# OpenDriveLab/kai0

Hardware: AMD Instinct MI355X
Metric: train samples/sec pi0.5 full FT (higher is better)
Workload: dtype bf16; 1 GPU; pi0.5 full fine-tune bf16, batch 32 per MI355X, 3-cam 224x224 (BASELINE.json configs[1]); global_batch=32, seq_len=1018, parallelism=dp1

## Files before the change

### include/kai0hip.h

```cpp
#ifndef KAI0HIP_H
#define KAI0HIP_H

#include <stdint.h>

#ifdef __cplusplus
extern "C" {
#endif

typedef void* kai0_stream_t;

const char* kai0_last_error(void);
int kai0_abi_version(void);
int kai0_device_info(int device, int* n_cu, int* lds_bytes, char* arch_name64);

typedef struct kai0_gemm_desc {
    const void* A;
    const void* B;
    void* C;
    int32_t M, N, K;
    int32_t a_kc, b_kc;
    int64_t lda, ldb, ldc;
    int32_t batch, batch_inner;
    int64_t sA1, sA2, sB1, sB2, sC1, sC2;
    int32_t a_rpb, b_rpb, c_rpb, _pad0;
// ... 5 lines not shown
    int32_t out_f32;
    void* pre_out;
    const void* gate;
    int32_t gate_rpb;
    int32_t accumulate;
    int64_t gate_ld;
    const void* residual;
    int64_t ldr;
    int64_t sR1, sR2;
    int32_t split_k;
    int32_t c_nontemporal;
    void* workspace;
    int64_t workspace_bytes;
    const void* aux1;
    const void* aux2;
    int32_t nseg, _pad2;
    struct {
        void* dst;
        int64_t ld;
        int32_t n_begin, _pad;
    } seg[3];
    const float* rowvec;
    int64_t rv_s1, rv_s2, rv_ld;
    const void* B2;
    void* pre_out2;
    void* norm_out;
    const void* norm_w;
    const void* norm_b;
    float norm_eps;
    int32_t norm_kind;
    const void* rope_cos;
    const void* rope_sin;
    int32_t rope_half, rope_n_end;
    int32_t persist, general_epilogue, small_w8, _pad3;
} kai0_gemm_desc;

int kai0_gemm_bf16(const kai0_gemm_desc* d, kai0_stream_t stream);
int kai0_gemm_desc_size(void);

#define KAI0_GEMM_LOOP_PLAIN2 0
#define KAI0_GEMM_LOOP_PLAIN4 1
#define KAI0_GEMM_LOOP_QUADRANT 2
#define KAI0_GEMM_LOOP_RING 3
#define KAI0_GEMM_LOOP_PERSISTENT 4
typedef struct kai0_gemm_plan_t {
    int32_t tile;
    int32_t waves;
    int32_t loop;
    int32_t tiles_m, tiles_n;
    int32_t k_chunk;
    int32_t simple_epilogue;
    int32_t _pad;
} kai0_gemm_plan_t;
int kai0_gemm_plan(const kai0_gemm_desc* d, kai0_gemm_plan_t* out);
int kai0_gemm_plan_size(void);

typedef struct kai0_skinny_seg {
    void* dst;
    int64_t ld;
    int32_t n_begin, n_end;
    int32_t rope, _pad;
} kai0_skinny_seg;

typedef struct kai0_skinny_desc {
    const void* A;
    const void* W;
    int64_t lda, ldw;
    int32_t M, N, K;
    int32_t pair_stride, mode, split_k;
    int32_t a_rpb, c_rpb;
    int64_t a_bs, a_off, c_bs, c_off;
    kai0_skinny_seg seg[3];
    int32_t nseg, gate_rpb;
    const void* gate;
    int64_t gate_ld;
    const void* residual;
    int64_t ldr;
    const float* rope_cos;
    const float* rope_sin;
    int32_t rope_half;
    int32_t w_packed;
    void* workspace;
    int64_t workspace_bytes;
    const float* mod;
    int64_t mod_ld;
// ... 233 lines not shown
```

### kai0_amd/_lib.py

```python

from __future__ import annotations

import ctypes as C
import os
import pathlib

_HERE = pathlib.Path(__file__).resolve().parent
LIB_PATH = _HERE / "lib" / "libkai0hip.so"
ABI_VERSION = 2

c_p = C.c_void_p
c_i = C.c_int
c_i64 = C.c_int64
c_f = C.c_float


class GemmSeg(C.Structure):
    _fields_ = [("dst", c_p), ("ld", c_i64), ("n_begin", C.c_int32), ("_pad", C.c_int32)]


class GemmDesc(C.Structure):

    _fields_ = [
        ("A", c_p), ("B", c_p), ("C", c_p),
        ("M", C.c_int32), ("N", C.c_int32), ("K", C.c_int32),
        ("a_kc", C.c_int32), ("b_kc", C.c_int32),
        ("lda", c_i64), ("ldb", c_i64), ("ldc", c_i64),
        ("batch", C.c_int32), ("batch_inner", C.c_int32),
        ("sA1", c_i64), ("sA2", c_i64), ("sB1", c_i64), ("sB2", c_i64), ("sC1", c_i64), ("sC2", c_i64),
        ("a_rpb", C.c_int32), ("b_rpb", C.c_int32), ("c_rpb", C.c_int32), ("_pad0", C.c_int32),
        ("a_bs", c_i64), ("a_off", c_i64), ("b_bs", c_i64), ("b_off", c_i64), ("c_bs", c_i64), ("c_off", c_i64),
        ("bias", c_p), ("bias_f32", C.c_int32), ("scale", c_f),
        ("act", C.c_int32), ("out_f32", C.c_int32),
        ("pre_out", c_p), ("gate", c_p), ("gate_rpb", C.c_int32), ("accumulate", C.c_int32),
        ("gate_ld", c_i64), ("residual", c_p), ("ldr", c_i64), ("sR1", c_i64), ("sR2", c_i64),
        ("split_k", C.c_int32), ("c_nontemporal", C.c_int32), ("workspace", c_p), ("workspace_bytes", c_i64),
        ("aux1", c_p), ("aux2", c_p),
        ("nseg", C.c_int32), ("_pad2", C.c_int32), ("seg", GemmSeg * 3),
        ("rowvec", c_p), ("rv_s1", c_i64), ("rv_s2", c_i64), ("rv_ld", c_i64),
        ("B2", c_p), ("pre_out2", c_p),
        ("norm_out", c_p), ("norm_w", c_p), ("norm_b", c_p), ("norm_eps", C.c_float), ("norm_kind", C.c_int32),
        ("rope_cos", c_p), ("rope_sin", c_p), ("rope_half", C.c_int32), ("rope_n_end", C.c_int32),
        ("persist", C.c_int32), ("general_epilogue", C.c_int32), ("small_w8", C.c_int32), ("_pad3", C.c_int32),
    ]


class GemmPlan(C.Structure):

    _fields_ = [("tile", C.c_int32), ("waves", C.c_int32), ("loop", C.c_int32), ("tiles_m", C.c_int32), ("tiles_n", C.c_int32),
                ("k_chunk", C.c_int32), ("simple_epilogue", C.c_int32), ("_pad", C.c_int32)]


GEMM_LOOPS = ("plain2", "plain4", "quadrant", "ring", "persistent")


class AttnDesc(C.Structure):

    _fields_ = [
        ("Q", c_p), ("K", c_p), ("V", c_p), ("O", c_p), ("P", c_p), ("qcode", c_p), ("kcode", c_p),
        ("rows", C.c_int32), ("Sk", C.c_int32), ("HD", C.c_int32), ("H", C.c_int32), ("q0", C.c_int32),
        ("batch", C.c_int32), ("batch_inner", C.c_int32), ("_pad0", C.c_int32),
        ("ldq", c_i64), ("ldk", c_i64), ("ldv", c_i64), ("ldo", c_i64), ("ldp", c_i64),
        ("sQ1", c_i64), ("sQ2", c_i64), ("sK1", c_i64), ("sK2", c_i64), ("sV1", c_i64), ("sV2", c_i64),
        ("sO1", c_i64), ("sO2", c_i64), ("sP", c_i64), ("qcode_ld", c_i64), ("kcode_ld", c_i64),
        ("scale", c_f), ("online", C.c_int32), ("lse", c_p), ("s_lse", c_i64),
    ]


class AttnBwdDesc(C.Structure):

    _fields_ = [
        ("dO", c_p), ("O", c_p), ("Q", c_p), ("K", c_p), ("V", c_p), ("lse", c_p), ("qcode", c_p), ("kcode", c_p),
        ("P", c_p), ("dS", c_p), ("dQ", c_p),
        ("batch", C.c_int32), ("rows", C.c_int32), ("Sk", C.c_int32), ("HD", C.c_int32), ("H", C.c_int32), ("_pad0", C.c_int32),
        ("ldo", c_i64), ("ldk", c_i64), ("ldv", c_i64), ("ldp", c_i64), ("sO", c_i64), ("sK", c_i64), ("sV", c_i64), ("sP", c_i64),
        ("s_lse", c_i64), ("qcode_ld", c_i64), ("kcode_ld", c_i64),
        ("scale", c_f), ("_pad1", C.c_int32),
    ]


class SkinnySeg(C.Structure):
    _fields_ = [("dst", c_p), ("ld", c_i64), ("n_begin", C.c_int32), ("n_end", C.c_int32), ("rope", C.c_int32),
                ("_pad", C.c_int32)]
# ... 185 lines not shown
```

### kai0_amd/csrc/gemm_bf16.hip

```cpp
#include "common.h"
#include "../../include/kai0hip.h"
#include <stdlib.h>
#include <algorithm>
#include <atomic>
#include <type_traits>

namespace {

constexpr int BK = 64;

#ifdef KAI0_ABLATE
#define KAI0_ABL(p) ((p).ablate)
#else
#define KAI0_ABL(p) 0
#endif

struct RowMap {
    int32_t rpb;
    int64_t bs, off;
    __device__ __forceinline__ int64_t operator()(int r) const {
        if (rpb == 0) return r;
        const int q = r / rpb;
        return (int64_t)q * bs + (r - q * rpb) + off;
    }
};

struct GemmArgs {
    const bf16_t* A;
    const bf16_t* B;
    void* C;
    int M, N, K;
    int64_t lda, ldb, ldc;
    int batch_inner;
    int64_t sA1, sA2, sB1, sB2, sC1, sC2;
    RowMap amap, bmap, cmap;
    const void* bias;
    int bias_f32;
    float scale;
    int act;
    int out_f32;
    bf16_t* pre_out;
    const bf16_t* aux1;
    const bf16_t* aux2;
    const bf16_t* gate;
    int gate_rpb;
    int accumulate;
    int64_t gate_ld;
    const bf16_t* residual;
    int64_t ldr, sR1, sR2;
    int tiles_m, tiles_n;
    int ablate;
    int nt_c;
    int simple_epi;
    int nt_pre;
    const float* rowvec;
    int64_t rv_s1, rv_s2, rv_ld;
    int nseg;
    bf16_t* seg_dst[3];
    int64_t seg_ld[3];
    int seg_begin[3];
    float* ws;
    int split_k, k_chunk;
    const bf16_t* B2;
    bf16_t* pre_out2;
    bf16_t* norm_out;
    const void* norm_w;
    const bf16_t* norm_b;
    float norm_eps;
    int norm_kind;
    const bf16_t* rope_cos;
    const bf16_t* rope_sin;
    int rope_half, rope_n_end;
};

typedef __attribute__((ext_vector_type(4))) int i32x4_t;
constexpr uint32_t OOB = 0x80000000u;
__device__ __forceinline__ void glds16(__amdgpu_buffer_rsrc_t rsrc, uint32_t voff, char* lds_dst_wave_uniform) {
    __builtin_amdgcn_raw_ptr_buffer_load_lds(rsrc, (LDS_PTR(void))lds_dst_wave_uniform, 16, (int)voff, 0, 0, 0);
}


__device__ __forceinline__ void store_pre8(bf16_t* dst, bf16x8 v, int nt) {
    if (nt) __builtin_nontemporal_store(v, reinterpret_cast<bf16x8*>(dst));
    else *reinterpret_cast<bf16x8*>(dst) = v;
}

// ... 1102 lines not shown
            lds_barrier();
            quad(I0{}, I0{});
            lds_barrier();
            read_b(tb, 1);
            __builtin_amdgcn_sched_barrier(0);
            issue_half(false, 1, t + 1);
            asm volatile("s_waitcnt vmcnt(8)" ::: "memory");
            lds_barrier();
            quad(I0{}, I1{});
            lds_barrier();
            read_a(ta, 1);
            __builtin_amdgcn_sched_barrier(0);
            issue_half(false, 0, t + 2);
            lds_barrier();
            quad(I1{}, I1{});
            lds_barrier();
            read_b(tb, 0);
            __builtin_amdgcn_sched_barrier(0);
            issue_half(true, 1, t + 2);
            asm volatile("s_waitcnt vmcnt(6)" ::: "memory");
            lds_barrier();
            quad(I1{}, I0{});
            lds_barrier();
        }
        asm volatile("s_waitcnt vmcnt(0)" ::: "memory");
        if (grp == 0) lds_barrier();
        lds_barrier();

        PS_STAMP(1);
        const int m0c = m0, n0c = n0;
        int nn = -1;
        unsigned raw = 0;
        if (tid == 0 && nxt >= 0) raw = draw();
        if (nxt >= 0) {
            setup(nxt);
            prologue_issue();
        }
        const int ccol = n0c + wn * 64 + (lane & 7) * 8;
        const bool col_ok = ccol < ((p.N + 7) & ~7);
        const bool fused_fast = p.act >= 2 && p.act <= 5 && p.bias == nullptr && p.gate == nullptr && p.residual == nullptr && !p.accumulate &&
                                !p.out_f32 && p.nseg == 0 && (p.act == 4 || p.scale == 1.0f) && (p.act != 3 || p.pre_out != nullptr);
        const bool simple_fast = SIMPLE_EPILOGUE_APPLIES(p.simple_epi, p.act, p.split_k, p.gate, p.out_f32, p.scale, p.cmap.rpb, p.N);
        auto to_slab = [&](int ti) {
            __builtin_amdgcn_wave_barrier();
#pragma unroll
            for (int j = 0; j < 4; ++j)
#pragma unroll
                for (int r = 0; r < 4; ++r) slab[(4 * g + r) * 64 + j * 16 + l15] = acc[ti][j][r];
            asm volatile("s_waitcnt lgkmcnt(0)" ::: "memory");
            __builtin_amdgcn_wave_barrier();
        };
        if (pair) {
            const int ocol = (n0c >> 1) + wn * 32 + (lane & 3) * 8;
            const bool ocol_ok = ocol < (p.N >> 1);
            bf16_t* cb = reinterpret_cast<bf16_t*>(p.C);
#pragma unroll
            for (int ti = 0; ti < MT; ++ti) {
                to_slab(ti);
                const int row = m0c + wm * 128 + ti * 16 + (lane >> 2);
                const float* sp = slab + (lane >> 2) * 64 + (lane & 3) * 8;
                const f32x4 g0 = *reinterpret_cast<const f32x4*>(sp), g1 = *reinterpret_cast<const f32x4*>(sp + 4);
                const f32x4 u0 = *reinterpret_cast<const f32x4*>(sp + 32), u1 = *reinterpret_cast<const f32x4*>(sp + 36);
                if (row < p.M && ocol_ok) {
                    const float gv[8] = {g0[0], g0[1], g0[2], g0[3], g1[0], g1[1], g1[2], g1[3]};
                    const float uv[8] = {u0[0], u0[1], u0[2], u0[3], u1[0], u1[1], u1[2], u1[3]};
                    bf16x8 gb, ub, hb;
#pragma unroll
                    for (int e = 0; e < 8; e += 2) {
                        const f32x2 gr = rbf2(f32x2{gv[e], gv[e + 1]}), ur = rbf2(f32x2{uv[e], uv[e + 1]});
                        const f32x2 hv = rbf2(gelu_tanh2(gr)) * ur;
                        gb[e] = f2bf(gr[0]); gb[e + 1] = f2bf(gr[1]);
                        ub[e] = f2bf(ur[0]); ub[e + 1] = f2bf(ur[1]);
                        hb[e] = f2bf(hv[0]); hb[e + 1] = f2bf(hv[1]);
                    }
                    const int64_t o = p.cmap(row) * p.ldc + ocol;
                    *reinterpret_cast<bf16x8*>(cb + o) = hb;
                    if (p.pre_out != nullptr) store_pre8(p.pre_out + o, gb, p.nt_pre);
                    if (p.pre_out2 != nullptr) store_pre8(p.pre_out2 + o, ub, p.nt_pre);
                }
            }
        } else if (fused_fast) {
            bf16_t* cb = reinterpret_cast<bf16_t*>(p.C);
#pragma unroll
            for (int h = 0; h < 2; ++h) {
                bf16x8 s0[8], s1[8];
                float ds[8];
                const int rbase = m0c + wm * 128 + h * 64 + (lane >> 3);
#pragma unroll
                for (int it = 0; it < 8; ++it) {
                    const int row = rbase + it * 8;
                    s0[it] = bf16x8{};
                    s1[it] = bf16x8{};
                    ds[it] = 0.f;
                    if (row < p.M && col_ok) {
                        const int64_t o = p.cmap(row) * p.ldc + ccol;
                        s0[it] = *reinterpret_cast<const bf16x8*>(p.aux1 + o);
                        if (p.act == 3) s1[it] = *reinterpret_cast<const bf16x8*>(p.aux2 + o);
                        if (p.act == 4) ds[it] = p.rowvec[(int64_t)row * p.rv_ld];
                    }
                }
#pragma unroll
                for (int i = 0; i < 4; ++i) {
                    to_slab(h * 4 + i);
#pragma unroll
                    for (int it2 = 0; it2 < 2; ++it2) {
                        const int it = 2 * i + it2;
                        const int row = rbase + it * 8;
                        const float* sp = slab + (it2 * 8 + (lane >> 3)) * 64 + (lane & 7) * 8;
                        const f32x4 v0 = *reinterpret_cast<const f32x4*>(sp), v1 = *reinterpret_cast<const f32x4*>(sp + 4);
                        const float v[8] = {v0[0], v0[1], v0[2], v0[3], v1[0], v1[1], v1[2], v1[3]};
                        if (row >= p.M || !col_ok) continue;
                        const int64_t o = p.cmap(row) * p.ldc + ccol;
                        bf16x8 ov;
                        if (p.act == 2) {
                            if (p.pre_out != nullptr) {
                                bf16x8 uv;
#pragma unroll
                                for (int e = 0; e < 8; ++e) uv[e] = f2bf(v[e]);
                                *reinterpret_cast<bf16x8*>(p.pre_out + o) = uv;
                            }
#pragma unroll
                            for (int e = 0; e < 8; e += 2) {
                                const f32x2 r = rbf2(gelu_tanh2(f32x2{bf2f(s0[it][e]), bf2f(s0[it][e + 1])})) * rbf2(f32x2{v[e], v[e + 1]});
                                ov[e] = f2bf(r[0]);
                                ov[e + 1] = f2bf(r[1]);
                            }
                        } else if (p.act == 3) {
                            bf16x8 du;
#pragma unroll
                            for (int e = 0; e < 8; e += 2) {
                                const f32x2 dh = rbf2(f32x2{v[e], v[e + 1]});
                                f32x2 gl, gr;
                                gelu_tanh_both2(f32x2{bf2f(s0[it][e]), bf2f(s0[it][e + 1])}, gl, gr);
                                const f32x2 a = dh * rbf2(gl);
                                const f32x2 b = rbf2(dh * f32x2{bf2f(s1[it][e]), bf2f(s1[it][e + 1])}) * gr;
                                du[e] = f2bf(a[0]); du[e + 1] = f2bf(a[1]);
                                ov[e] = f2bf(b[0]); ov[e + 1] = f2bf(b[1]);
                            }
                            *reinterpret_cast<bf16x8*>(p.pre_out + o) = du;
                        } else if (p.act == 5) {
#pragma unroll
                            for (int e = 0; e < 8; e += 2) {
                                f32x2 gl, gr;
                                gelu_tanh_both2(f32x2{bf2f(s0[it][e]), bf2f(s0[it][e + 1])}, gl, gr);
                                const f32x2 b = rbf2(f32x2{v[e], v[e + 1]}) * gr;
                                ov[e] = f2bf(b[0]); ov[e + 1] = f2bf(b[1]);
                            }
                        } else {
#pragma unroll
                            for (int e = 0; e < 8; ++e) ov[e] = f2bf((bf2f(s0[it][e]) * (v[e] - ds[it])) * p.scale);
                        }
                        *reinterpret_cast<bf16x8*>(cb + o) = ov;
                    }
                }
            }
        } else if (simple_fast) {
            const bool has_bias = p.bias != nullptr, has_res = p.residual != nullptr, gelu = p.act == 1;
            const int M_ = p.M, nt_pre_ = p.nt_pre, nt_c_ = p.nt_c;
            const bf16_t* res_ = p.residual;
            bf16_t* pre_ = p.pre_out;
            const int64_t ldr_ = p.ldr, ldc_ = p.ldc;
            float bv[8] = {0.f, 0.f, 0.f, 0.f, 0.f, 0.f, 0.f, 0.f};
            if (has_bias && col_ok) {
                if (p.bias_f32) {
                    const f32x4 b0 = *reinterpret_cast<const f32x4*>(reinterpret_cast<const float*>(p.bias) + ccol);
                    const f32x4 b1 = *reinterpret_cast<const f32x4*>(reinterpret_cast<const float*>(p.bias) + ccol + 4);
#pragma unroll
                    for (int e = 0; e < 4; ++e) { bv[e] = b0[e]; bv[4 + e] = b1[e]; }
                } else {
                    const bf16x8 b = *reinterpret_cast<const bf16x8*>(reinterpret_cast<const bf16_t*>(p.bias) + ccol);
#pragma unroll
                    for (int e = 0; e < 8; ++e) bv[e] = bf2f(b[e]);
                }
            }
            bf16_t* cl = reinterpret_cast<bf16_t*>(p.C) + ccol;
            int64_t ldl = p.ldc;
            if (p.nseg > 0) {
                cl = p.seg_dst[0] + (ccol - p.seg_begin[0]);
                ldl = p.seg_ld[0];
                if (p.nseg > 1 && ccol >= p.seg_begin[1]) {
                    cl = p.seg_dst[1] + (ccol - p.seg_begin[1]);
                    ldl = p.seg_ld[1];
                }
                if (p.nseg > 2 && ccol >= p.seg_begin[2]) {
                    cl = p.seg_dst[2] + (ccol - p.seg_begin[2]);
// ... 263 lines not shown
    return -3;
}

}

#ifdef KAI0_PS_TRACE
KAI0_API int kai0_debug_ps_trace(long long* host_out) {
    return (int)hipMemcpyFromSymbol(host_out, HIP_SYMBOL(g_ps_trace), sizeof(long long) * 256 * 8);
}
#endif

static int gemm_validate(const kai0_gemm_desc* d) {
    KAI0_REQUIRE(d != nullptr, "kai0_gemm_bf16: null descriptor");
    KAI0_REQUIRE(d->M > 0 && d->N > 0 && d->K > 0, "kai0_gemm_bf16: empty problem M=%d N=%d K=%d", d->M, d->N,
                 d->K);
    KAI0_REQUIRE(d->A && d->B && d->C, "kai0_gemm_bf16: null operand");
    KAI0_REQUIRE((d->lda % 8) == 0 && (d->ldb % 8) == 0 && (d->ldc % 8) == 0,
                 "kai0_gemm_bf16: leading dims must be multiples of 8 (lda=%lld ldb=%lld ldc=%lld)",
                 (long long)d->lda, (long long)d->ldb, (long long)d->ldc);
    KAI0_REQUIRE((d->N % 8) == 0 || (d->b_kc && d->ldc >= ((d->N + 7) & ~7) && !d->bias && !d->gate && !d->residual &&
                                     !d->pre_out && !d->accumulate),
                 "kai0_gemm_bf16: N=%d not a multiple of 8 needs b_kc, padded C rows and a plain epilogue", d->N);
    KAI0_REQUIRE((d->K % 8) == 0 || (!d->a_kc && !d->b_kc), "kai0_gemm_bf16: K=%d must be a multiple of 8 for "
                 "K-contiguous operands", d->K);
    KAI0_REQUIRE(d->a_kc || (d->M % 8) == 0, "kai0_gemm_bf16: M=%d must be a multiple of 8 when A is [K][M]",
                 d->M);
    KAI0_REQUIRE(((uintptr_t)d->A % 16) == 0 && ((uintptr_t)d->B % 16) == 0 && ((uintptr_t)d->C % 16) == 0,
                 "kai0_gemm_bf16: operands must be 16-byte aligned");
    KAI0_REQUIRE(d->batch <= 1 || (((d->sA1 | d->sA2 | d->sB1 | d->sB2) & 7) == 0 && ((d->sC1 | d->sC2) & (d->out_f32 ? 3 : 7)) == 0),
                 "kai0_gemm_bf16: batch strides must be multiples of 8 elements (16 B)");
    KAI0_REQUIRE(d->gate == nullptr || d->gate_rpb > 0, "kai0_gemm_bf16: gate needs gate_rpb > 0");
    KAI0_REQUIRE(d->act >= 0 && d->act <= 7, "kai0_gemm_bf16: unknown act %d", d->act);
    KAI0_REQUIRE(d->persist >= 0 && d->persist <= 2 && d->small_w8 >= 0 && d->small_w8 <= 2 && d->general_epilogue >= 0 &&
                     d->general_epilogue <= 1,
                 "kai0_gemm_bf16: hook out of range (persist=%d, small_w8=%d: 0..2; general_epilogue=%d: 0..1)", d->persist, d->small_w8,
                 d->general_epilogue);
    KAI0_REQUIRE(d->act != 7 || (d->rope_cos && d->rope_sin && d->rope_half == 128 && d->rope_n_end > 0 && (d->rope_n_end % 256) == 0 &&
                                 d->rope_n_end <= d->N && (d->N % 128) == 0 && d->a_kc && d->b_kc && d->batch <= 1 && d->split_k <= 1 &&
                                 !d->out_f32 && !d->accumulate && !d->bias && !d->gate && !d->residual && !d->pre_out &&
                                 (d->scale == 0.0f || d->scale == 1.0f) && d->b_rpb == 0 && ((uintptr_t)d->rope_cos % 16) == 0 &&
                                 ((uintptr_t)d->rope_sin % 16) == 0),
                 "kai0_gemm_bf16: act=7 (RoPE epilogue) needs bf16 cos / sin tables [M][128], rope_n_end %% 256 == 0, N %% 128 == 0, K-contiguous "
                 "operands, one batch entry, no split-K, a plain bf16 output");
    KAI0_REQUIRE(d->act != 6 || (d->B2 && d->a_kc && d->b_kc && d->batch <= 1 && d->split_k <= 1 && !d->out_f32 && !d->accumulate &&
                                 d->nseg == 0 && !d->bias && !d->gate && !d->residual && (d->scale == 0.0f || d->scale == 1.0f) &&
                                 (d->N % 32) == 0 && d->b_rpb == 0 && ((uintptr_t)d->B2 % 16) == 0),
                 "kai0_gemm_bf16: act=6 (GeGLU pair) needs B2 = up weight, K-contiguous operands, N %% 32 == 0, one batch entry, a "
                 "plain bf16 output");
    KAI0_REQUIRE(d->norm_kind == 0 ||
                     ((d->norm_kind == 1 || d->norm_kind == 2) && d->split_k > 1 && d->norm_out && d->norm_w && (d->norm_kind == 1 || d->norm_b) &&
                      d->batch <= 1 && !d->out_f32 && d->nseg == 0 && (d->N % 8) == 0 && d->N <= 2048 && d->act == 0 && !d->gate &&
                      !d->rowvec && ((uintptr_t)d->norm_out % 16) == 0 && ((uintptr_t)d->norm_w % 16) == 0),
                 "kai0_gemm_bf16: a fused norm (norm_kind=%d) needs split_k > 1, norm_out / norm_w (/ norm_b), one batch entry, a plain "
                 "bf16 output with N %% 8 == 0, N <= 2048, no activation / gate", d->norm_kind);
    KAI0_REQUIRE(d->act != 5 || (d->aux1 && !d->out_f32 && !d->accumulate && d->nseg == 0 && (d->N % 8) == 0),
                 "kai0_gemm_bf16: act=5 (fused GELU backward) needs aux1 = pre-activation, plain bf16 output");
    KAI0_REQUIRE(d->act != 4 || (d->aux1 && d->rowvec && !d->out_f32 && !d->accumulate && d->nseg == 0 && (d->N % 8) == 0),
                 "kai0_gemm_bf16: act=4 (fused softmax backward) needs aux1 = P, rowvec = D, plain bf16 output");
    KAI0_REQUIRE(d->act < 2 || d->act >= 4 || ((d->pre_out || d->act == 2) && d->aux1 && (d->act == 2 || d->aux2) && !d->out_f32 && (d->N % 8) == 0),
                 "kai0_gemm_bf16: act=%d (fused GeGLU) needs pre_out and aux inputs, bf16 output", d->act);
    KAI0_REQUIRE(d->nseg >= 0 && d->nseg <= 3, "kai0_gemm_bf16: nseg=%d", d->nseg);
    if (d->nseg > 0) {
        KAI0_REQUIRE(!d->out_f32 && !d->accumulate && (d->batch <= 1) && (d->act < 2 || d->act == 7) && !d->pre_out && (d->N % 8) == 0,
                     "kai0_gemm_bf16: column segments need a plain bf16 epilogue, batch 1");
        KAI0_REQUIRE(d->act != 4, "kai0_gemm_bf16: column segments and act=4 are exclusive");
        for (int i = 0; i < d->nseg; ++i)
            KAI0_REQUIRE(d->seg[i].dst && (d->seg[i].ld % 8) == 0 && (d->seg[i].n_begin % 8) == 0 &&
                             ((uintptr_t)d->seg[i].dst % 16) == 0 && d->seg[i].n_begin == (i ? d->seg[i].n_begin : 0) &&
                             (i == 0 || d->seg[i].n_begin > d->seg[i - 1].n_begin),
// ... 16 lines not shown
    }
    return 0;
}

static kai0_gemm_plan_t gemm_select(const kai0_gemm_desc* d) {
    kai0_gemm_plan_t pl{};
    const int batch = d->batch > 0 ? d->batch : 1;
    const int split = d->split_k > 1 ? d->split_k : 1;
    const int N = d->act == 6 ? 2 * d->N : d->N;
    const int k_chunk = split > 1 ? ((d->K + split - 1) / split + BK - 1) / BK * BK : d->K;
    const int64_t big_tiles = (int64_t)((d->M + 255) / 256) * ((N + 255) / 256) * batch * split;
    const bool big = d->act != 7 && big_tiles >= 160 && d->K >= 256;
    const int64_t small_blocks = (int64_t)((d->M + 127) / 128) * ((N + 127) / 128) * batch * split;
    const bool deep = small_blocks <= 256 && k_chunk >= 256;
    const bool w8 = !big && d->a_kc && d->b_kc && (d->act <= 1 || d->act == 7) && (d->small_w8 == 2 || (d->small_w8 == 0 && deep));
    const int persist = d->persist == 1 ? 0 : (d->persist == 2 ? 2 : 1);
    const bool ps_ok = persist && big && d->a_kc && d->b_kc && batch == 1 && split == 1 &&
                       big_tiles >= (persist == 2 ? 512 : 2048) &&
                       (d->K % 8) == 0 && !d->rowvec && d->a_rpb == 0 && d->b_rpb == 0;
    const bool ps_rule = N >= 8192 || d->K >= 8192;
    pl.tile = big ? 256 : 128;
    pl.waves = big || w8 ? 8 : 4;
    if (ps_ok && (persist == 2 || ps_rule)) pl.loop = KAI0_GEMM_LOOP_PERSISTENT;
    else if (big && d->a_kc && d->b_kc) pl.loop = KAI0_GEMM_LOOP_QUADRANT;
    else if (big && !d->a_kc && !d->b_kc) pl.loop = KAI0_GEMM_LOOP_RING;
    else if (big) pl.loop = KAI0_GEMM_LOOP_PLAIN2;
    else if (w8 || deep) pl.loop = KAI0_GEMM_LOOP_PLAIN4;
    else pl.loop = KAI0_GEMM_LOOP_PLAIN2;
    pl.tiles_m = (d->M + pl.tile - 1) / pl.tile;
    pl.tiles_n = (N + pl.tile - 1) / pl.tile;
    pl.k_chunk = k_chunk;
    pl.simple_epilogue = big && SIMPLE_EPILOGUE_APPLIES(d->general_epilogue == 0, d->act, split, d->gate, d->out_f32,
                                                        (d->scale == 0.0f ? 1.0f : d->scale), d->c_rpb, N);
    return pl;
}

KAI0_API int kai0_gemm_plan_size(void) { return (int)sizeof(kai0_gemm_plan_t); }

KAI0_API int kai0_gemm_plan(const kai0_gemm_desc* d, kai0_gemm_plan_t* out) {
    KAI0_REQUIRE(out != nullptr, "kai0_gemm_plan: null result");
    if (int rc = gemm_validate(d)) return rc;
    *out = gemm_select(d);
    return 0;
}

KAI0_API int kai0_gemm_bf16(const kai0_gemm_desc* d, kai0_stream_t stream) {
    if (int rc = gemm_validate(d)) return rc;
    const int batch = d->batch > 0 ? d->batch : 1;
    GemmArgs p;
    p.A = (const bf16_t*)d->A;
    p.B = (const bf16_t*)d->B;
    p.C = d->C;
    p.M = d->M; p.N = d->act == 6 ? 2 * d->N : d->N; p.K = d->K;
    p.B2 = (const bf16_t*)d->B2;
    p.pre_out2 = (bf16_t*)d->pre_out2;
    p.norm_out = (bf16_t*)d->norm_out;
    p.norm_w = d->norm_w;
    p.norm_b = (const bf16_t*)d->norm_b;
    p.norm_eps = d->norm_eps;
    p.norm_kind = d->norm_kind;
    p.rope_cos = (const bf16_t*)d->rope_cos;
    p.rope_sin = (const bf16_t*)d->rope_sin;
    p.rope_half = d->rope_half;
    p.rope_n_end = d->rope_n_end;
    p.lda = d->lda; p.ldb = d->ldb; p.ldc = d->ldc;
    p.batch_inner = d->batch_inner > 0 ? d->batch_inner : 1;
    p.sA1 = d->sA1; p.sA2 = d->sA2; p.sB1 = d->sB1; p.sB2 = d->sB2; p.sC1 = d->sC1; p.sC2 = d->sC2;
    p.amap = RowMap{d->a_rpb, d->a_bs, d->a_off};
    p.bmap = RowMap{d->b_rpb, d->b_bs, d->b_off};
    p.cmap = RowMap{d->c_rpb, d->c_bs, d->c_off};
    p.bias = d->bias; p.bias_f32 = d->bias_f32;
    p.scale = d->scale == 0.0f ? 1.0f : d->scale;
    p.act = d->act; p.out_f32 = d->out_f32;
    p.pre_out = (bf16_t*)d->pre_out;
    p.aux1 = (const bf16_t*)d->aux1;
    p.aux2 = (const bf16_t*)d->aux2;
    p.gate = (const bf16_t*)d->gate; p.gate_rpb = d->gate_rpb; p.gate_ld = d->gate_ld;
    p.accumulate = d->accumulate;
    p.residual = (const bf16_t*)d->residual; p.ldr = d->ldr; p.sR1 = d->sR1; p.sR2 = d->sR2;
#ifdef KAI0_ABLATE
    static const int ablate = [] { const char* e = getenv("KAI0_GEMM_ABLATE"); return e ? atoi(e) : 0; }();
    p.ablate = ablate;
#else
    p.ablate = 0;
#endif
    p.nt_pre = 1;
    p.nt_c = d->c_nontemporal != 0;
    p.simple_epi = d->general_epilogue == 0;
    p.rowvec = d->rowvec; p.rv_s1 = d->rv_s1; p.rv_s2 = d->rv_s2; p.rv_ld = d->rv_ld;
    p.nseg = d->nseg;
    for (int i = 0; i < 3; ++i) {
        p.seg_dst[i] = i < d->nseg ? (bf16_t*)d->seg[i].dst : nullptr;
        p.seg_ld[i] = i < d->nseg ? d->seg[i].ld : 0;
        p.seg_begin[i] = i < d->nseg ? d->seg[i].n_begin : 0;
    }
    const kai0_gemm_plan_t pl = gemm_select(d);
    const int split = d->split_k > 1 ? d->split_k : 1;
    p.split_k = split;
    p.k_chunk = pl.k_chunk;
    p.ws = split > 1 ? (float*)d->workspace : nullptr;
    hipStream_t s = (hipStream_t)stream;
    int rc;
    if (pl.loop == KAI0_GEMM_LOOP_PERSISTENT) {
        const int64_t big_tiles = (int64_t)pl.tiles_m * pl.tiles_n;
        constexpr int LDS = 2 * 2 * 256 * 64 * 2 + 8 * 4096;
        struct PsDev { unsigned int* ctr = nullptr; int cus = 0; };
        static PsDev ps_dev[64];
        static std::atomic<unsigned> next_slot{0};
        int dv = 0;
        KAI0_REQUIRE(hipGetDevice(&dv) == hipSuccess && dv >= 0 && dv < 64, "kai0_gemm_bf16: hipGetDevice");
        PsDev& pd = ps_dev[dv];
        if (pd.ctr == nullptr) {
            void* sym = nullptr;
            hipError_t e = hipGetSymbolAddress(&sym, HIP_SYMBOL(g_ps_ctr));
            if (e == hipSuccess) e = hipFuncSetAttribute((const void*)gemm_nt_persistent_kernel, hipFuncAttributeMaxDynamicSharedMemorySize, LDS);
            hipDeviceProp_t pr;
            if (e == hipSuccess) e = hipGetDeviceProperties(&pr, dv);
            KAI0_REQUIRE(e == hipSuccess, "kai0_gemm_bf16: persistent kernel setup failed: %s", hipGetErrorString(e));
            pd.cus = pr.multiProcessorCount > 0 ? pr.multiProcessorCount : 256;
            pd.ctr = (unsigned int*)sym;
        }
        unsigned int* ctr_base = pd.ctr;
        p.tiles_m = (d->M + 255) / 256;
        p.tiles_n = (p.N + 255) / 256;
        const int nblk = (int)std::min<int64_t>(big_tiles, pd.cus);
        unsigned int* ctr = ctr_base + (size_t)(next_slot.fetch_add(1) % PS_SLOTS) * 16;
        hipLaunchKernelGGL(gemm_nt_persistent_kernel, dim3(nblk), dim3(512), LDS, s, p, ctr);
        return kai0_check_launch("kai0_gemm_bf16 (persistent)");
    }
// ... 21 lines not shown
```

### kai0_amd/ops.py

```python

from __future__ import annotations

import contextlib
import ctypes as C
import os
import math

import torch

from . import _lib
from ._lib import AttnBwdDesc, AttnDesc, GemmDesc

BF16 = torch.bfloat16
F32 = torch.float32

NORM_PARTIAL_BLOCKS = 512
COLSUM_BLOCKS = 256


def _stream() -> int:
    return torch.cuda.current_stream().cuda_stream


def _p(t: torch.Tensor | None) -> int | None:
    return None if t is None else t.data_ptr()


def _chk(t: torch.Tensor, dtype, name: str) -> None:
    if not t.is_cuda:
        raise _lib.Kai0HipError(f"{name}: expected a CUDA (HIP) tensor; the product path has no CPU fallback")
    if t.dtype != dtype:
        raise TypeError(f"{name}: expected {dtype}, got {t.dtype}")
    if not t.is_contiguous():
        raise ValueError(f"{name}: expected a contiguous tensor")


GEMM_TUNING = {"persist": {"0": 1, "2": 2}.get(os.environ.get("KAI0_GEMM_PERSIST", "1"), 0), "general_epilogue": 0,
               "small_w8": {"0": 1, "2": 2}.get(os.environ.get("KAI0_GEMM_W8", "1"), 0)}


@contextlib.contextmanager
def gemm_tuning(**kw):
    unknown = set(kw) - set(GEMM_TUNING)
    if unknown:
        raise KeyError(f"gemm_tuning: unknown hook(s) {sorted(unknown)}")
    old = dict(GEMM_TUNING)
    GEMM_TUNING.update(kw)
    try:
        yield
    finally:
        GEMM_TUNING.update(old)


def gemm(
    A: torch.Tensor, B: torch.Tensor, out: torch.Tensor, *, M: int, N: int, K: int, a_kc: bool = True,
    b_kc: bool = True, lda: int, ldb: int, ldc: int, batch: int = 1, batch_inner: int = 1,
    sA=(0, 0), sB=(0, 0), sC=(0, 0), a_map=None, b_map=None, c_map=None, bias: torch.Tensor | None = None,
    scale: float = 1.0, act: int = 0, pre_out: torch.Tensor | None = None, gate: torch.Tensor | None = None,
    gate_rpb: int = 0, gate_ld: int = 0, residual: torch.Tensor | None = None, ldr: int = 0, sR=(0, 0),
    accumulate: bool = False, a_off_elems: int = 0, b_off_elems: int = 0, c_off_elems: int = 0, split_k: int = 1,
    aux1: torch.Tensor | None = None, aux2: torch.Tensor | None = None, segs=None, rowvec=None, rv=(0, 0, 1),
    B2: torch.Tensor | None = None, pre_out2: torch.Tensor | None = None, norm=None, nt_out: bool = False, rope=None,
    _plan: "_lib.GemmPlan | None" = None,
) -> torch.Tensor:
    for t in (A, B, out):
        if not t.is_cuda:
            raise _lib.Kai0HipError("gemm: expected CUDA (HIP) tensors; the product path has no CPU fallback")
    if A.dtype != BF16 or B.dtype != BF16:
        raise TypeError(f"gemm: bf16 operands expected, got {A.dtype} / {B.dtype}")
    d = GemmDesc()
    d.A = A.data_ptr() + 2 * a_off_elems
# ... 34 lines not shown
    if gate is not None:
        d.gate = gate.data_ptr()
        d.gate_rpb = gate_rpb
        d.gate_ld = gate_ld
    if residual is not None:
        d.residual = residual.data_ptr()
        d.ldr = ldr
        d.sR1, d.sR2 = sR
    d.accumulate = int(accumulate)
    d.c_nontemporal = int(nt_out)
    if rowvec is not None:
        if rowvec.dtype != F32:
            raise TypeError("gemm: rowvec must be f32")
        d.rowvec = rowvec.data_ptr()
        d.rv_s1, d.rv_s2, d.rv_ld = rv
    if segs:
        d.nseg = len(segs)
        for i, (dst, ld, nb) in enumerate(segs):
            d.seg[i].dst, d.seg[i].ld, d.seg[i].n_begin = dst.data_ptr(), ld, nb
    if split_k > 1 and _plan is not None:
        d.split_k, d.workspace, d.workspace_bytes = split_k, d.A, batch * split_k * M * N * 4
    elif split_k > 1:
        ws = _workspace(batch * split_k * M * N * 4, A.device)
        d.split_k, d.workspace, d.workspace_bytes = split_k, ws.data_ptr(), ws.numel()
    if norm is not None:
        kind, nout, nw, nb, neps = norm
        _chk(nout, BF16, "gemm: norm_out")
        _chk(nw, F32 if kind == 1 else BF16, "gemm: norm weight")
        d.norm_kind, d.norm_out, d.norm_w, d.norm_eps = int(kind), nout.data_ptr(), nw.data_ptr(), float(neps)
        if nb is not None:
            _chk(nb, BF16, "gemm: norm bias")
            d.norm_b = nb.data_ptr()
    d.persist, d.general_epilogue, d.small_w8 = GEMM_TUNING["persist"], GEMM_TUNING["general_epilogue"], GEMM_TUNING["small_w8"]
    if _plan is not None:
        _lib.call("kai0_gemm_plan", C.byref(d), C.byref(_plan))
        return out
    _lib.call("kai0_gemm_bf16", C.byref(d), _stream())
    return out


def gemm_plan(A: torch.Tensor, B: torch.Tensor, out: torch.Tensor, **kw) -> dict:
    pl = _lib.GemmPlan()
    gemm(A, B, out, _plan=pl, **kw)
    return {"tile": pl.tile, "waves": pl.waves, "loop": _lib.GEMM_LOOPS[pl.loop], "tiles_m": pl.tiles_m, "tiles_n": pl.tiles_n,
            "k_chunk": pl.k_chunk, "simple_epilogue": bool(pl.simple_epilogue)}


def skinny_split_k(N: int, K: int) -> int:
    if K % 512:
        raise _lib.Kai0HipError(f"skinny gemm: K={K} must be a multiple of 512")
    tiles = N // 32
    if K % 1024 == 0 and tiles * (K // 1024) >= 190:
        return K // 1024
    return K // 512


def skinny_workspace(M: int, N: int, split_k: int, device) -> torch.Tensor:
    return torch.empty((max(split_k, 1), M, N), dtype=F32, device=device)


def skinny_gemm(A, W, *, M: int, N: int, K: int, lda: int, ldw: int, mode: int = 0, pair_stride: int = 16, segs=None,
                split_k: int = 1, workspace=None, a_map=None, c_map=None, gate=None, gate_rpb: int = 0, gate_ld: int = 0,
                residual=None, ldr: int = 0, rope_cos=None, rope_sin=None, rope_half: int = 0, mod=None, mod_ld: int = 0,
                mod_rpb: int = 0, eps: float = 1e-6, w_packed: bool = False, rowsq_in=None, rowsq_parts: int = 0, cvec=None,
                rowsq_out=None):
    for t in (A, W):
        if not t.is_cuda or t.dtype != BF16:
            raise _lib.Kai0HipError("skinny_gemm: expected bf16 CUDA (HIP) tensors; the product path has no CPU fallback")
    d = _lib.SkinnyDesc()
    d.A, d.W, d.lda, d.ldw = A.data_ptr(), W.data_ptr(), lda, ldw
    d.M, d.N, d.K = M, N, K
    d.pair_stride, d.mode, d.split_k = pair_stride, mode, split_k
    d.w_packed = int(w_packed)
    if a_map:
        d.a_rpb, d.a_bs, d.a_off = a_map
    if c_map:
        d.c_rpb, d.c_bs, d.c_off = c_map
    d.nseg = len(segs or ())
# ... 1490 lines not shown
```

Before: 67.22 samples/s.

## Prefetch fused-epilogue aux operands into LDS ahead of next tile prologue

In the persistent GEMM loop, fused GELU-type epilogues (act 2/3/5) can now load their aux operands asynchronously into per-wave LDS windows with buffer loads. The first pass is issued before the next tile's prologue, and later passes are software-pipelined with vmcnt waits, instead of reading the operands into registers. The aim is to hide the latency of the epilogue operand reads and to reduce register pressure. The epilogue arithmetic is factored into a shared lambda. This adds fragile hand-tuned waitcnt counts and reuses LDS regions that must not conflict with the next tile's prologue loads.

New measurement: 67.67 samples/s, median of 6. No clear change (+0.7%).

```diff
diff --git a/include/kai0hip.h b/include/kai0hip.h
--- a/include/kai0hip.h
+++ b/include/kai0hip.h
@@ -61,7 +61,7 @@
     const void* rope_cos;
     const void* rope_sin;
     int32_t rope_half, rope_n_end;
-    int32_t persist, general_epilogue, small_w8, _pad3;
+    int32_t persist, general_epilogue, small_w8, epi_operands;
 } kai0_gemm_desc;
 
 int kai0_gemm_bf16(const kai0_gemm_desc* d, kai0_stream_t stream);
@@ -79,7 +79,7 @@
     int32_t tiles_m, tiles_n;
     int32_t k_chunk;
     int32_t simple_epilogue;
-    int32_t _pad;
+    int32_t epi_lds;
 } kai0_gemm_plan_t;
 int kai0_gemm_plan(const kai0_gemm_desc* d, kai0_gemm_plan_t* out);
 int kai0_gemm_plan_size(void);
diff --git a/kai0_amd/_lib.py b/kai0_amd/_lib.py
--- a/kai0_amd/_lib.py
+++ b/kai0_amd/_lib.py
@@ -48,7 +48,7 @@
 class GemmPlan(C.Structure):
 
     _fields_ = [("tile", C.c_int32), ("waves", C.c_int32), ("loop", C.c_int32), ("tiles_m", C.c_int32), ("tiles_n", C.c_int32),
-                ("k_chunk", C.c_int32), ("simple_epilogue", C.c_int32), ("_pad", C.c_int32)]
+                ("k_chunk", C.c_int32), ("simple_epilogue", C.c_int32), ("epi_lds", C.c_int32)]
 
 
 GEMM_LOOPS = ("plain2", "plain4", "quadrant", "ring", "persistent")
diff --git a/kai0_amd/csrc/gemm_bf16.hip b/kai0_amd/csrc/gemm_bf16.hip
--- a/kai0_amd/csrc/gemm_bf16.hip
+++ b/kai0_amd/csrc/gemm_bf16.hip
@@ -52,6 +52,7 @@
     int ablate;
     int nt_c;
     int simple_epi;
+    int epi_lds;
     int nt_pre;
     const float* rowvec;
     int64_t rv_s1, rv_s2, rv_ld;
@@ -1220,15 +1221,34 @@
         int nn = -1;
         unsigned raw = 0;
         if (tid == 0 && nxt >= 0) raw = draw();
-        if (nxt >= 0) {
-            setup(nxt);
-            prologue_issue();
-        }
         const int ccol = n0c + wn * 64 + (lane & 7) * 8;
         const bool col_ok = ccol < ((p.N + 7) & ~7);
         const bool fused_fast = p.act >= 2 && p.act <= 5 && p.bias == nullptr && p.gate == nullptr && p.residual == nullptr && !p.accumulate &&
                                 !p.out_f32 && p.nseg == 0 && (p.act == 4 || p.scale == 1.0f) && (p.act != 3 || p.pre_out != nullptr);
         const bool simple_fast = SIMPLE_EPILOGUE_APPLIES(p.simple_epi, p.act, p.split_k, p.gate, p.out_f32, p.scale, p.cmap.rpb, p.N);
+        const bool epi_lds = fused_fast && p.epi_lds != 0;
+        const bool two_ops = p.act == 3;
+        const int r0w = m0c + wm * 128;
+        const int vsteps = (n0c + wn * 64 < ((p.N + 7) & ~7)) ? min(16, max(0, (p.M - r0w + 7) >> 3)) : 0;
+        const __amdgpu_buffer_rsrc_t x1_rsrc = __builtin_amdgcn_make_buffer_rsrc((void*)(epi_lds ? p.aux1 : p.A), 0, (int)OOB, 0x00020000);
+        const __amdgpu_buffer_rsrc_t x2_rsrc = __builtin_amdgcn_make_buffer_rsrc((void*)(epi_lds && two_ops ? p.aux2 : p.A), 0, (int)OOB, 0x00020000);
+        char* win = smem + STAGE + (wave < 4 ? 8192 + (wave >> 1) * 16384 + (wave & 1) * 4096 : A_TILE + (wave - 4) * 8192);
+        auto aux_issue = [&](int pass) {
+#pragma unroll
+            for (int st = 0; st < 2; ++st) {
+                const int row = r0w + pass * 16 + st * 8 + (lane >> 3);
+                const uint32_t off = (row < p.M && col_ok) ? (uint32_t)((p.cmap(row) * p.ldc + ccol) * 2) : OOB;
+                glds16(x1_rsrc, off, win + st * 1024);
+                if (two_ops) glds16(x2_rsrc, off, win + 2048 + st * 1024);
+            }
+        };
+        __builtin_amdgcn_sched_barrier(0);
+        if (epi_lds && vsteps > 0) aux_issue(0);
+        __builtin_amdgcn_sched_barrier(0);
+        if (nxt >= 0) {
+            setup(nxt);
+            prologue_issue();
+        }
         auto to_slab = [&](int ti) {
             __builtin_amdgcn_wave_barrier();
 #pragma unroll
@@ -1238,10 +1258,52 @@
             asm volatile("s_waitcnt lgkmcnt(0)" ::: "memory");
             __builtin_amdgcn_wave_barrier();
         };
+        bf16_t* cb = reinterpret_cast<bf16_t*>(p.C);
+        auto fused_store = [&](int64_t o, const float (&v)[8], bf16x8 g8, bf16x8 u8, float dsum) {
+            bf16x8 ov;
+            if (p.act == 2) {
+                if (p.pre_out != nullptr) {
+                    bf16x8 uv;
+#pragma unroll
+                    for (int e = 0; e < 8; ++e) uv[e] = f2bf(v[e]);
+                    *reinterpret_cast<bf16x8*>(p.pre_out + o) = uv;
+                }
+#pragma unroll
+                for (int e = 0; e < 8; e += 2) {
+                    const f32x2 r = rbf2(gelu_tanh2(f32x2{bf2f(g8[e]), bf2f(g8[e + 1])})) * rbf2(f32x2{v[e], v[e + 1]});
+                    ov[e] = f2bf(r[0]);
+                    ov[e + 1] = f2bf(r[1]);
+                }
+            } else if (p.act == 3) {
+                bf16x8 du;
+#pragma unroll
+                for (int e = 0; e < 8; e += 2) {
+                    const f32x2 dh = rbf2(f32x2{v[e], v[e + 1]});
+                    f32x2 gl, gr;
+                    gelu_tanh_both2(f32x2{bf2f(g8[e]), bf2f(g8[e + 1])}, gl, gr);
+                    const f32x2 a = dh * rbf2(gl);
+                    const f32x2 b = rbf2(dh * f32x2{bf2f(u8[e]), bf2f(u8[e + 1])}) * gr;
+                    du[e] = f2bf(a[0]); du[e + 1] = f2bf(a[1]);
+                    ov[e] = f2bf(b[0]); ov[e + 1] = f2bf(b[1]);
+                }
+                *reinterpret_cast<bf16x8*>(p.pre_out + o) = du;
+            } else if (p.act == 5) {
+#pragma unroll
+                for (int e = 0; e < 8; e += 2) {
+                    f32x2 gl, gr;
+                    gelu_tanh_both2(f32x2{bf2f(g8[e]), bf2f(g8[e + 1])}, gl, gr);
+                    const f32x2 b = rbf2(f32x2{v[e], v[e + 1]}) * gr;
+                    ov[e] = f2bf(b[0]); ov[e + 1] = f2bf(b[1]);
+                }
+            } else {
+#pragma unroll
+                for (int e = 0; e < 8; ++e) ov[e] = f2bf((bf2f(g8[e]) * (v[e] - dsum)) * p.scale);
+            }
+            *reinterpret_cast<bf16x8*>(cb + o) = ov;
+        };
         if (pair) {
             const int ocol = (n0c >> 1) + wn * 32 + (lane & 3) * 8;
             const bool ocol_ok = ocol < (p.N >> 1);
-            bf16_t* cb = reinterpret_cast<bf16_t*>(p.C);
 #pragma unroll
             for (int ti = 0; ti < MT; ++ti) {
                 to_slab(ti);
@@ -1267,8 +1329,40 @@
                     if (p.pre_out2 != nullptr) store_pre8(p.pre_out2 + o, ub, p.nt_pre);
                 }
             }
+        } else if (epi_lds) {
+            const int sps = two_ops || (p.act == 2 && p.pre_out != nullptr) ? 2 : 1;
+#pragma unroll
+            for (int ti = 0; ti < MT; ++ti) {
+                if (2 * ti >= vsteps) continue;
+                to_slab(ti);
+                if (ti == 0) {
+                    if (nxt >= 0) asm volatile("s_waitcnt vmcnt(12)" ::: "memory");
+                    else asm volatile("s_waitcnt vmcnt(0)" ::: "memory");
+                } else {
+                    if (sps == 2) asm volatile("s_waitcnt vmcnt(4)" ::: "memory");
+                    else asm volatile("s_waitcnt vmcnt(2)" ::: "memory");
+                }
+                bf16x8 g8[2], u8[2];
+#pragma unroll
+                for (int st = 0; st < 2; ++st) {
+                    g8[st] = *reinterpret_cast<const bf16x8*>(win + st * 1024 + lane * 16);
+                    u8[st] = two_ops ? *reinterpret_cast<const bf16x8*>(win + 2048 + st * 1024 + lane * 16) : bf16x8{};
+                }
+                asm volatile("s_waitcnt lgkmcnt(0)" ::: "memory");
+                __builtin_amdgcn_sched_barrier(0);
+                if (ti + 1 < MT && 2 * (ti + 1) < vsteps) aux_issue(ti + 1);
+                __builtin_amdgcn_sched_barrier(0);
+#pragma unroll
+                for (int st = 0; st < 2; ++st) {
+                    const int row = r0w + ti * 16 + st * 8 + (lane >> 3);
+                    const float* sp = slab + (st * 8 + (lane >> 3)) * 64 + (lane & 7) * 8;
+                    const f32x4 v0 = *reinterpret_cast<const f32x4*>(sp), v1 = *reinterpret_cast<const f32x4*>(sp + 4);
+                    const float v[8] = {v0[0], v0[1], v0[2], v0[3], v1[0], v1[1], v1[2], v1[3]};
+                    if (row >= p.M || !col_ok) continue;
+                    fused_store(p.cmap(row) * p.ldc + ccol, v, g8[st], u8[st], 0.f);
+                }
+            }
         } else if (fused_fast) {
-            bf16_t* cb = reinterpret_cast<bf16_t*>(p.C);
 #pragma unroll
             for (int h = 0; h < 2; ++h) {
                 bf16x8 s0[8], s1[8];
@@ -1299,46 +1393,7 @@
                         const float v[8] = {v0[0], v0[1], v0[2], v0[3], v1[0], v1[1], v1[2], v1[3]};
                         if (row >= p.M || !col_ok) continue;
                         const int64_t o = p.cmap(row) * p.ldc + ccol;
-                        bf16x8 ov;
-                        if (p.act == 2) {
-                            if (p.pre_out != nullptr) {
-                                bf16x8 uv;
-#pragma unroll
-                                for (int e = 0; e < 8; ++e) uv[e] = f2bf(v[e]);
-                                *reinterpret_cast<bf16x8*>(p.pre_out + o) = uv;
-                            }
-#pragma unroll
-                            for (int e = 0; e < 8; e += 2) {
-                                const f32x2 r = rbf2(gelu_tanh2(f32x2{bf2f(s0[it][e]), bf2f(s0[it][e + 1])})) * rbf2(f32x2{v[e], v[e + 1]});
-                                ov[e] = f2bf(r[0]);
-                                ov[e + 1] = f2bf(r[1]);
-                            }
-                        } else if (p.act == 3) {
-                            bf16x8 du;
-#pragma unroll
-                            for (int e = 0; e < 8; e += 2) {
-                                const f32x2 dh = rbf2(f32x2{v[e], v[e + 1]});
-                                f32x2 gl, gr;
-                                gelu_tanh_both2(f32x2{bf2f(s0[it][e]), bf2f(s0[it][e + 1])}, gl, gr);
-                                const f32x2 a = dh * rbf2(gl);
-                                const f32x2 b = rbf2(dh * f32x2{bf2f(s1[it][e]), bf2f(s1[it][e + 1])}) * gr;
-                                du[e] = f2bf(a[0]); du[e + 1] = f2bf(a[1]);
-                                ov[e] = f2bf(b[0]); ov[e + 1] = f2bf(b[1]);
-                            }
-                            *reinterpret_cast<bf16x8*>(p.pre_out + o) = du;
-                        } else if (p.act == 5) {
-#pragma unroll
-                            for (int e = 0; e < 8; e += 2) {
-                                f32x2 gl, gr;
-                                gelu_tanh_both2(f32x2{bf2f(s0[it][e]), bf2f(s0[it][e + 1])}, gl, gr);
-                                const f32x2 b = rbf2(f32x2{v[e], v[e + 1]}) * gr;
-                                ov[e] = f2bf(b[0]); ov[e + 1] = f2bf(b[1]);
-                            }
-                        } else {
-#pragma unroll
-                            for (int e = 0; e < 8; ++e) ov[e] = f2bf((bf2f(s0[it][e]) * (v[e] - ds[it])) * p.scale);
-                        }
-                        *reinterpret_cast<bf16x8*>(cb + o) = ov;
+                        fused_store(o, v, s0[it], s1[it], ds[it]);
                     }
                 }
             }
@@ -1668,9 +1723,9 @@
     KAI0_REQUIRE(d->gate == nullptr || d->gate_rpb > 0, "kai0_gemm_bf16: gate needs gate_rpb > 0");
     KAI0_REQUIRE(d->act >= 0 && d->act <= 7, "kai0_gemm_bf16: unknown act %d", d->act);
     KAI0_REQUIRE(d->persist >= 0 && d->persist <= 2 && d->small_w8 >= 0 && d->small_w8 <= 2 && d->general_epilogue >= 0 &&
-                     d->general_epilogue <= 1,
-                 "kai0_gemm_bf16: hook out of range (persist=%d, small_w8=%d: 0..2; general_epilogue=%d: 0..1)", d->persist, d->small_w8,
-                 d->general_epilogue);
+                     d->general_epilogue <= 1 && d->epi_operands >= 0 && d->epi_operands <= 1,
+                 "kai0_gemm_bf16: hook out of range (persist=%d, small_w8=%d: 0..2; general_epilogue=%d, epi_operands=%d: 0..1)", d->persist,
+                 d->small_w8, d->general_epilogue, d->epi_operands);
     KAI0_REQUIRE(d->act != 7 || (d->rope_cos && d->rope_sin && d->rope_half == 128 && d->rope_n_end > 0 && (d->rope_n_end % 256) == 0 &&
                                  d->rope_n_end <= d->N && (d->N % 128) == 0 && d->a_kc && d->b_kc && d->batch <= 1 && d->split_k <= 1 &&
                                  !d->out_f32 && !d->accumulate && !d->bias && !d->gate && !d->residual && !d->pre_out &&
@@ -1753,6 +1808,13 @@
     pl.k_chunk = k_chunk;
     pl.simple_epilogue = big && SIMPLE_EPILOGUE_APPLIES(d->general_epilogue == 0, d->act, split, d->gate, d->out_f32,
                                                         (d->scale == 0.0f ? 1.0f : d->scale), d->c_rpb, N);
+    {
+        const int64_t c_rows = d->c_rpb ? ((int64_t)(d->M / d->c_rpb) + 1) * d->c_bs + d->c_off : d->M;
+        const bool fused = (d->act == 2 || d->act == 3 || d->act == 5) && !d->bias && !d->gate && !d->residual && !d->accumulate &&
+                           !d->out_f32 && d->nseg == 0 && (d->scale == 0.0f || d->scale == 1.0f) && (d->act != 3 || d->pre_out);
+        pl.epi_lds = pl.loop == KAI0_GEMM_LOOP_PERSISTENT && fused && d->epi_operands == 0 && d->c_bs >= 0 && d->c_off >= 0 &&
+                     c_rows * d->ldc * 2 < (int64_t)0x7FFF0000;
+    }
     return pl;
 }
 
@@ -1808,6 +1870,7 @@
     p.nt_pre = 1;
     p.nt_c = d->c_nontemporal != 0;
     p.simple_epi = d->general_epilogue == 0;
+    p.epi_lds = 0;
     p.rowvec = d->rowvec; p.rv_s1 = d->rv_s1; p.rv_s2 = d->rv_s2; p.rv_ld = d->rv_ld;
     p.nseg = d->nseg;
     for (int i = 0; i < 3; ++i) {
@@ -1816,6 +1879,7 @@
         p.seg_begin[i] = i < d->nseg ? d->seg[i].n_begin : 0;
     }
     const kai0_gemm_plan_t pl = gemm_select(d);
+    p.epi_lds = pl.epi_lds;
     const int split = d->split_k > 1 ? d->split_k : 1;
     p.split_k = split;
     p.k_chunk = pl.k_chunk;
diff --git a/kai0_amd/ops.py b/kai0_amd/ops.py
--- a/kai0_amd/ops.py
+++ b/kai0_amd/ops.py
@@ -37,6 +37,19 @@
 
 GEMM_TUNING = {"persist": {"0": 1, "2": 2}.get(os.environ.get("KAI0_GEMM_PERSIST", "1"), 0), "general_epilogue": 0,
                "small_w8": {"0": 1, "2": 2}.get(os.environ.get("KAI0_GEMM_W8", "1"), 0)}
+
+
+EPI_OPERANDS = [0]
+
+
+@contextlib.contextmanager
+def epilogue_operands(mode: int):
+    old = EPI_OPERANDS[0]
+    EPI_OPERANDS[0] = int(mode)
+    try:
+        yield
+    finally:
+        EPI_OPERANDS[0] = old
 
 
 @contextlib.contextmanager
@@ -137,6 +150,7 @@
             _chk(nb, BF16, "gemm: norm bias")
             d.norm_b = nb.data_ptr()
     d.persist, d.general_epilogue, d.small_w8 = GEMM_TUNING["persist"], GEMM_TUNING["general_epilogue"], GEMM_TUNING["small_w8"]
+    d._pad3 = EPI_OPERANDS[0]
     if _plan is not None:
         _lib.call("kai0_gemm_plan", C.byref(d), C.byref(_plan))
         return out
@@ -149,6 +163,12 @@
     gemm(A, B, out, _plan=pl, **kw)
     return {"tile": pl.tile, "waves": pl.waves, "loop": _lib.GEMM_LOOPS[pl.loop], "tiles_m": pl.tiles_m, "tiles_n": pl.tiles_n,
             "k_chunk": pl.k_chunk, "simple_epilogue": bool(pl.simple_epilogue)}
+
+
+def gemm_epilogue_operands(A: torch.Tensor, B: torch.Tensor, out: torch.Tensor, **kw) -> str:
+    pl = _lib.GemmPlan()
+    gemm(A, B, out, _plan=pl, **kw)
+    return "lds" if pl.epi_lds else "registers"
 
 
 def skinny_split_k(N: int, K: int) -> int:
```
